# nyenyu12/BioInformatics-project-for-Shotgun-Metagenomics-Pseudo-alignment-shotgun-

Hardware: AMD Instinct MI355X
Metric: reads/sec pseudo-aligned (k=31, 150bp) at 1/2/4/8 GPUs; % HBM roofline (higher is better)
Workload: dtype u8

## Files before the change

### bioinformatics-project-for-shotgun-metagenomics-pseudo-alignment-shotgun-_amd/csrc/pa_align.hip

```cpp
#include <hip/hip_runtime.h>

#include <algorithm>
#include <cstdio>
#include <cstdlib>
#include <cstring>
#include <vector>

#include "pa_device.h"
#include "pa_internal.h"

using namespace pad;

namespace {

constexpr int kBlock = 256;
constexpr int kWaves = kBlock / 64;
constexpr uint32_t kSegMaxWaves = 16384;
constexpr uint64_t kSegSlack = 64ull * kSegMaxWaves;
constexpr uint32_t kLdsGenomeCap = 2048;

enum : uint32_t { F_MRQ = 1, F_MKQ = 2, F_MG = 4 };

struct AlignArgs {
    const void *table;
    uint64_t cap;
    HomeCfg home;
    uint32_t G;
    int k;
    const uint32_t *class_genomes;
    const uint64_t *class_mask;
    const uint32_t *tile_cls;
    const uint64_t *tile_pk;
    uint64_t tile_n;
    const uint64_t *goff;
    const uint64_t *tile_lw;
    const uint64_t *tile_big;
    const void *tile_nb;
    uint64_t nb_base1, nb_split;
    const uint32_t *nbbig_ld;
    uint64_t nbbig_mask;
    int nb_spec;
// ... 21 lines not shown
    unsigned long long *stats;
    unsigned long long *uniq;
    unsigned long long *amb;
    unsigned long long *first;
    uint32_t *queue;
    unsigned long long *qcount;
    unsigned long long *deferred_total;
    uint32_t *queue_hard;
    unsigned long long *queue_hard_count;
    uint32_t *queue_na;
    unsigned long long *queue_na_count;
    uint64_t *queue_na_keys;
    uint32_t *queue_rc;
    uint64_t *queue_rc_anc;
    unsigned long long *queue_rc_count;
    uint32_t *queue_na2;
    unsigned long long *queue_na2_count;
    uint64_t na_min;
    uint32_t na_seg;
    uint32_t *seg_cnt;
    uint32_t nseg;
    uint64_t seg_cap;
    uint64_t queue_cap;
    const uint4 *qmask;
    const uint8_t *qdrop;
    const uint32_t *rlist;
    const unsigned long long *rlist_count;
    unsigned long long *dbg;
};

__device__ __forceinline__ uint64_t first_key(uint64_t read, uint32_t rank) { return (read << 20) | rank; }


struct WgCounters {
    uint32_t *uniq;
    uint32_t *amb;
    unsigned long long *first;
    bool lds;
};

__device__ __forceinline__ void count_genome(const AlignArgs &a, const WgCounters &c, uint32_t g, bool unique,
                                             uint32_t times, uint64_t key) {
    if (c.lds) {
        atomicAdd(unique ? &c.uniq[g] : &c.amb[g], times);
        if (key < c.first[g]) atomicMin(&c.first[g], (unsigned long long)key);
    } else {
// ... 106 lines not shown
    }
    switch (k >> 2) {
        case 0: quality_reads<0>(qual, off, n, k, T, mrq, flags, qmask, qdrop); break;
        case 1: quality_reads<1>(qual, off, n, k, T, mrq, flags, qmask, qdrop); break;
        case 2: quality_reads<2>(qual, off, n, k, T, mrq, flags, qmask, qdrop); break;
        case 3: quality_reads<3>(qual, off, n, k, T, mrq, flags, qmask, qdrop); break;
        case 4: quality_reads<4>(qual, off, n, k, T, mrq, flags, qmask, qdrop); break;
        case 5: quality_reads<5>(qual, off, n, k, T, mrq, flags, qmask, qdrop); break;
        case 6: quality_reads<6>(qual, off, n, k, T, mrq, flags, qmask, qdrop); break;
        case 7: quality_reads<7>(qual, off, n, k, T, mrq, flags, qmask, qdrop); break;
        case 8: quality_reads<8>(qual, off, n, k, T, mrq, flags, qmask, qdrop); break;
        case 9: quality_reads<9>(qual, off, n, k, T, mrq, flags, qmask, qdrop); break;
        case 10: quality_reads<10>(qual, off, n, k, T, mrq, flags, qmask, qdrop); break;
        case 11: quality_reads<11>(qual, off, n, k, T, mrq, flags, qmask, qdrop); break;
        case 12: quality_reads<12>(qual, off, n, k, T, mrq, flags, qmask, qdrop); break;
        case 13: quality_reads<13>(qual, off, n, k, T, mrq, flags, qmask, qdrop); break;
        case 14: quality_reads<14>(qual, off, n, k, T, mrq, flags, qmask, qdrop); break;
        case 15: quality_reads<15>(qual, off, n, k, T, mrq, flags, qmask, qdrop); break;
        default: break;
    }
}

#include "pa_lane.h"

__global__ __launch_bounds__(256) void k_tile_big(const uint32_t *__restrict__ tile_cls, uint64_t n, uint32_t G,
                                                  const uint32_t *__restrict__ class_genomes, int32_t mg,
                                                  uint64_t *__restrict__ big, uint64_t n_words) {
    const uint32_t lane = threadIdx.x & 63;
    const uint64_t nw = (uint64_t)gridDim.x * (blockDim.x >> 6);
    for (uint64_t j = (uint64_t)blockIdx.x * (blockDim.x >> 6) + (threadIdx.x >> 6); j < n_words; j += nw) {
        const uint64_t t = 64 * j + lane;
        const uint32_t v = t < n ? tile_cls[t] : NONE;
        const bool ok = v != NONE && (int64_t)class_size_of(v & ~PA_TILE_REP, G, class_genomes) > (int64_t)mg;
        const uint64_t b = __ballot(ok);
        if (lane == 0) big[j] = b;
    }
}


__global__ __launch_bounds__(256) void k_nb_merge(const uint64_t *__restrict__ nb, const uint32_t *__restrict__ nbbig,
                                                  uint64_t n_words, uint4 *__restrict__ out) {
    const uint64_t stride = (uint64_t)gridDim.x * blockDim.x;
    for (uint64_t i = (uint64_t)blockIdx.x * blockDim.x + threadIdx.x; i < n_words; i += stride) {
        const uint64_t v = nb[i];
        out[i] = make_uint4((uint32_t)v, (uint32_t)(v >> 32), nbbig[i], 0u);
    }
// ... 427 lines not shown
    hipStream_t st;
    int slot;
    hipEvent_t e0 = nullptr;
    KernelTimer(pa_index *i, hipStream_t s, int sl) : idx(i), st(s), slot(sl) {
        if (idx && idx->profile && hipEventCreate(&e0) == hipSuccess) hipEventRecord(e0, st);
    }
    ~KernelTimer() {
        hipEvent_t e1 = nullptr;
        if (e0 && hipEventCreate(&e1) == hipSuccess && hipEventRecord(e1, st) == hipSuccess)
            idx->kev.push_back({slot, e0, e1});
        else if (e0)
            hipEventDestroy(e0);
    }
};

constexpr uint64_t kRcnbMinReads = 32768;
pa_status launch_lane(const AlignArgs &a0, hipStream_t st, pa_index *prof = nullptr, bool long_reads = false,
                      int nw = 1) {
    const bool need_q = (a0.prm.flags & (F_MRQ | F_MKQ)) != 0;
    const bool win_q = (a0.prm.flags & F_MKQ) != 0;
    const bool mg = (a0.prm.flags & F_MG) != 0;
    const bool nm4 = long_reads && !win_q && nw == 1;
    AlignArgs a = a0;
    const size_t shm = lane_lds_bytes(a.G, nm4 ? 4 : 2);
    auto kern = nw == 3
                    ? (win_q ? (mg ? k_align_lane<true, true, true, 2, 3> : k_align_lane<true, true, false, 2, 3>)
                       : need_q ? (mg ? k_align_lane<true, false, true, 2, 3> : k_align_lane<true, false, false, 2, 3>)
                                : (mg ? k_align_lane<false, false, true, 2, 3> : k_align_lane<false, false, false, 2, 3>))
              : nw == 2
                    ? (win_q ? (mg ? k_align_lane<true, true, true, 2, 2> : k_align_lane<true, true, false, 2, 2>)
                       : need_q ? (mg ? k_align_lane<true, false, true, 2, 2> : k_align_lane<true, false, false, 2, 2>)
                                : (mg ? k_align_lane<false, false, true, 2, 2> : k_align_lane<false, false, false, 2, 2>))
              : nm4 ? (need_q ? (mg ? k_align_lane<true, false, true, 4> : k_align_lane<true, false, false, 4>)
                              : (mg ? k_align_lane<false, false, true, 4> : k_align_lane<false, false, false, 4>))
              : win_q ? (mg ? k_align_lane<true, true, true> : k_align_lane<true, true, false>)
              : need_q ? (mg ? k_align_lane<true, false, true> : k_align_lane<true, false, false>)
                       : (mg ? k_align_lane<false, false, true> : k_align_lane<false, false, false>);
    if (shm > 64 * 1024) PA_HIP(hipFuncSetAttribute((const void *)kern, hipFuncAttributeMaxDynamicSharedMemorySize, (int)shm));
    int per_cu = 0, dev = 0, cus = 256;
    PA_HIP(hipOccupancyMaxActiveBlocksPerMultiprocessor(&per_cu, kern, kBlock, shm));
    PA_HIP(hipGetDevice(&dev));
    PA_HIP(hipDeviceGetAttribute(&cus, hipDeviceAttributeMultiprocessorCount, dev));
    const uint64_t want = (a.n + kBlock - 1) / kBlock;
    const uint64_t resident = (uint64_t)std::max(1, per_cu) * (uint64_t)cus;
    const unsigned grid = (unsigned)std::max<uint64_t>(1, std::min<uint64_t>(want, resident));
    {
        const char *e = std::getenv("PA_NA_SEG");
        const uint64_t waves = (uint64_t)grid * kWaves, chunks = (a.n + 63) / 64;
        a.nseg = (uint32_t)waves;
        a.seg_cap = 64 * ((chunks + waves - 1) / waves);
        a.na_seg = a.queue_na && a.queue_na_keys && a.seg_cnt && !nm4 && nw == 1 && waves <= kSegMaxWaves &&
                   waves * a.seg_cap <= a.queue_cap && !(e && e[0] == '0');
    }
    {
        KernelTimer kt(prof, st, PA_PROF_LANE);
        hipLaunchKernelGGL(kern, dim3(grid), dim3(kBlock), shm, st, a);
        PA_HIP(hipGetLastError());
    }
    if (a.queue_na) {
        AlignArgs b = a;
        if (prof && prof->rcnb_pending && a.queue_na_keys) {
            unsigned long long c = 0;
            PA_HIP(hipMemcpyAsync(&c, a.queue_na_count, 8, hipMemcpyDeviceToHost, st));
            PA_HIP(hipStreamSynchronize(st));
            if (c >= std::max<uint64_t>(kRcnbMinReads, a.n / 64)) {
                PA_TRY(pa::index_build_rcnb(prof, st));
                const char *e = std::getenv("PA_NA_RCNB");
                if (!(e && e[0] == '0')) b.tile_rcnb = prof->tile_rcnb;
            } else if (++prof->rcnb_checks >= 2) {
                prof->rcnb_pending = 0;
            }
        }
        if (a.queue_na_keys) {
// ... 179 lines not shown
}

pa_status reserve_queues(pa_index *idx, uint64_t n) {
    if (!idx->seg_cnt) PA_HIP(pa::dev_malloc(&idx->seg_cnt, (uint64_t)kSegMaxWaves * 4));
    n += kSegSlack;
    if (idx->queue_cap >= n) return PA_OK;
    pa::dev_free(idx->queue);
    pa::dev_free(idx->queue_hard);
    pa::dev_free(idx->queue_na);
    pa::dev_free(idx->queue_na2);
    pa::dev_free(idx->queue_na_keys);
    pa::dev_free(idx->queue_rc);
    pa::dev_free(idx->queue_rc_anc);
    idx->queue = idx->queue_hard = idx->queue_na = idx->queue_na2 = idx->queue_rc = nullptr;
    idx->queue_na_keys = idx->queue_rc_anc = nullptr;
    idx->queue_cap = 0;
    PA_HIP(pa::dev_malloc(&idx->queue, n * 4));
    PA_HIP(pa::dev_malloc(&idx->queue_hard, n * 4));
    PA_HIP(pa::dev_malloc(&idx->queue_na, n * 4));
    PA_HIP(pa::dev_malloc(&idx->queue_na2, n * 4));
    PA_HIP(pa::dev_malloc(&idx->queue_na_keys, n * 16));
    PA_HIP(pa::dev_malloc(&idx->queue_rc, n * 4));
    PA_HIP(pa::dev_malloc(&idx->queue_rc_anc, n * 8));
    if (!idx->na_count) PA_HIP(pa::dev_malloc(&idx->na_count, 24));
    idx->queue_cap = n;
    return PA_OK;
}

__global__ __launch_bounds__(256) void k_reads_qstats(const uint8_t *__restrict__ qual,
                                                      const uint64_t *__restrict__ off, uint64_t n, uint32_t *out) {
    typedef unsigned short us2 __attribute__((ext_vector_type(2)));
    const uint64_t tid = (uint64_t)blockIdx.x * blockDim.x + threadIdx.x, stride = (uint64_t)gridDim.x * blockDim.x;
    const uint64_t b0 = off[0], b1 = off[n];
    const uint64_t mis = (uint64_t)(uintptr_t)qual & 15;
    const uint64_t a0 = min(b1, ((b0 + mis + 15) & ~15ull) - mis), a1 = max(a0, ((b1 + mis) & ~15ull) - mis);
    uint32_t qm = 255, lm = 0xFFFFFFFFu;
    if (tid < 16) {
        if (b0 + tid < a0) qm = min(qm, (uint32_t)qual[b0 + tid]);
        if (a1 + tid < b1) qm = min(qm, (uint32_t)qual[a1 + tid]);
    }
    us2 mlo = {255, 255}, mhi = {255, 255};
    const uint4 *vp = (const uint4 *)(qual + a0);
    const uint64_t nv = (a1 - a0) >> 4;
    auto fold = [&](const uint4 x) {
        const uint32_t d[4] = {x.x, x.y, x.z, x.w};
#pragma unroll
        for (int j = 0; j < 4; j++) {
// ... 166 lines not shown
                hipLaunchKernelGGL(idx->k > 63 ? k_quality_masks<true> : k_quality_masks<false>, dim3((unsigned)std::min<uint64_t>((r->n + 255) / 256, 65536)),
                                   dim3(256), 0, st, r->qual, r->off, r->n, (int)idx->k, (int64_t)a.prm.mrq,
                                   (int64_t)a.prm.mkq, a.prm.flags & (F_MRQ | F_MKQ), idx->qmask, idx->qdrop);
                PA_HIP(hipGetLastError());
                a.qmask = idx->qmask;
                a.qdrop = idx->qdrop;
            }
            bool na = a.bloom != nullptr;
            if (const char *e = std::getenv("PA_LANE_NOANCHOR")) na = e[0] == '1';
            if (idx->nw > 3) na = false;
            a.queue_na = na ? idx->queue_na : nullptr;
            a.queue_na_count = idx->na_count;
            const bool rcw = na && a.tile_rcp && a.bloom;
            a.queue_na_keys = rcw ? idx->queue_na_keys : nullptr;
            a.queue_rc = idx->queue_rc;
            a.queue_rc_anc = idx->queue_rc_anc;
            a.queue_rc_count = idx->na_count + 1;
            a.seg_cnt = idx->seg_cnt;
            a.queue_cap = idx->queue_cap;
            a.queue_na2 = idx->queue_na2;
            a.queue_na2_count = idx->na_count + 2;
            a.na_min = 32768;
            if (const char *e = std::getenv("PA_NA_MIN")) a.na_min = std::strtoull(e, nullptr, 10);
            if (na) PA_HIP(hipMemsetAsync(idx->na_count, 0, 24, st));
            const bool long_reads = r->max_len > (uint32_t)kLaneMaxLen ||
                                    (r->max_len >= idx->k && r->max_len - idx->k + 1 > (uint32_t)kLaneMaxW);
            PA_TRY(launch_lane(a, st, idx, long_reads, idx->nw));
            a.rlist = idx->queue_hard;
            a.rlist_count = a.queue_hard_count;
        }
        {
            KernelTimer kt(idx, st, PA_PROF_WAVE);
            PA_TRY(idx->nw == 1   ? launch_fast_wpl<1>(a, wpl, st)
                   : idx->nw == 2 ? launch_fast_wpl<2>(a, wpl, st)
                   : idx->nw == 3 ? launch_fast_wpl<3>(a, wpl, st)
                                  : launch_fast_wpl<4>(a, wpl, st));
        }
        if (idx->profile) {
            PA_HIP(hipEventRecord(e1, st));
            idx->ev_start.push_back(e0);
            idx->ev_stop.push_back(e1);
        }
        x.a = a;
        x.use_queue = 1;
    } else {
        x.use_queue = 0;
    }
// ... 113 lines not shown
```

### bioinformatics-project-for-shotgun-metagenomics-pseudo-alignment-shotgun-_amd/csrc/pa_lane.h

```cpp

constexpr uint64_t kPosMask = (1ull << 40) - 1;
template <int NM>
struct LaneShape {
    static constexpr int MAXW = 64 * NM;
    static constexpr int NWD = NM == 2 ? 6 : 9;
    static constexpr int MAXLEN = 32 * NWD - 16;
    static constexpr int NB = NM + 1;
};
constexpr int kLaneMaxW = LaneShape<2>::MAXW;
constexpr int kLaneMaxLen = LaneShape<2>::MAXLEN;
constexpr int kLaneWords = LaneShape<2>::NWD;
#ifndef PA_LANE_MAXMIS
#define PA_LANE_MAXMIS 40
#endif
constexpr uint32_t kLaneMaxMis = PA_LANE_MAXMIS;
#ifndef PA_LANE_PROBES
#define PA_LANE_PROBES 4
#endif
#ifndef PA_LANE_SEEDS
#define PA_LANE_SEEDS 5
#endif
#ifndef PA_SEED_SLOTS
#define PA_SEED_SLOTS 2
#endif
#ifndef PA_LANE_RANK_WORDS
#define PA_LANE_RANK_WORDS 6
#endif
#ifndef PA_LANE_SLOTS
#define PA_LANE_SLOTS 1
#endif
constexpr int kPassEntries = 64 * PA_LANE_PROBES;
#ifndef PA_TWO_WINQ
#define PA_TWO_WINQ 1
#endif
#ifndef PA_LANE_LDS_GENOMES
#define PA_LANE_LDS_GENOMES 1664
#endif
constexpr uint32_t kLaneLdsGenomeCap = PA_LANE_LDS_GENOMES;

template <int NM>
struct __align__(16) LaneWave {
    uint64_t R[64][LaneShape<NM>::NWD + 1];
    unsigned long long cand[64];
    uint32_t flags[64];
    uint32_t hr[64];
    uint32_t gsp[64];
    uint16_t list[kPassEntries];
    uint32_t again_r[128];
    unsigned long long again_a[128];
};

enum : int {
    LANE_UNIQUE = 0, LANE_AMB = 1, LANE_UNMAPPED = 2, LANE_DROP = 3, LANE_HARD = 4, LANE_WALK = 5, LANE_AGAIN = 6,
    LANE_NOANCHOR = 7
};

template <int N>
__device__ __forceinline__ uint64_t word_at(const uint64_t (&v)[N], uint32_t q) {
    uint64_t r = 0;
#pragma unroll
    for (int i = 0; i < N; i++) r = (q == (uint32_t)i) ? v[i] : r;
// ... 203 lines not shown
    }
}

template <int NWD = kLaneWords>
__device__ __forceinline__ uint32_t lane_count_mismatches(const uint64_t *row, uint32_t len, uint64_t A,
                                                          const uint64_t (&gw)[NWD + 1]) {
    const uint32_t gr = (uint32_t)(2 * A & 63);
    uint32_t n = 0;
    const uint32_t qlast = (len - 1) >> 5, rl = len - 32 * qlast;
    const uint64_t tail = rl >= 32 ? ~0ull : ~0ull << (64 - 2 * rl);
#pragma unroll
    for (int i = 0; i < NWD; i++) {
        if (32 * i >= (int)len) break;
        const uint64_t gwi = gr ? ((gw[i] << gr) | (gw[i + 1] >> (64 - gr))) : gw[i];
        uint64_t d = row[i] ^ gwi;
        if ((uint32_t)i == qlast) d &= tail;
        n += __popcll((d | (d >> 1)) & 0x5555555555555555ull);
    }
    return n;
}

__device__ __forceinline__ bool lane_fits(const AlignArgs &a, uint32_t len, int64_t A) {
    return A >= 0 && (uint64_t)A + len <= a.tile_n;
}

template <int NM, bool NEED_Q, bool WIN_Q, bool SEEDS = true, int NW = 1>
__device__ __forceinline__ void lane_prep(const AlignArgs &a, uint64_t r, unsigned long long cd, uint64_t *row,
                                          LaneRead<NM> &S) {
    using SH = LaneShape<NM>;
    static_assert(NM == 2 || !WIN_Q, "the window-quality masks cover 128 windows");
    constexpr int NWD = SH::NWD;
    S.kind = LANE_HARD;
    S.hr = S.nspec = S.nincl = 0;
#pragma unroll
    for (int i = 0; i < NM; i++) S.F[i] = 0;
    S.qf = 0;
    S.uoff = 0;
    const int k = a.k;
    const uint32_t flags = a.prm.flags;
    const uint64_t o = a.off[r];
    const uint32_t len = (uint32_t)(a.off[r + 1] - o);
    const uint64_t o0 = o & ~15ull;
    const uint32_t shift = (uint32_t)(o & 15);
    S.len = len;
    if (len > (uint32_t)SH::MAXLEN) return (void)LANE_HARD_WHY(0);
    if (NEED_Q) {
// ... 256 lines not shown
    uint64_t gw[kLaneWords + 1], pa3[3], pb3[3];
    lane_blocks<true>(a, Ac, len, gw, pa3, pb3);
    const uint32_t g = S.acls < a.G ? S.acls : genome_of(a.goff, a.gblk, atp);
    S.g = g;
    const uint64_t gs = a.goff[g], ge = a.goff[g + 1];
    if (!in_tile || A < (int64_t)gs || (uint64_t)A + W - 1 + k > ge) {
        S.kind = LANE_HARD;
        return (void)LANE_HARD_WHY(4);
    }
    const uint32_t fr = (uint32_t)(Ac & 63);
    const uint64_t PA0 = fr ? (pa3[0] >> fr) | (pa3[1] << (64 - fr)) : pa3[0];
    const uint64_t PA1 = fr ? (pa3[1] >> fr) | (pa3[2] << (64 - fr)) : pa3[1];
    const uint64_t PB0 = fr ? (pb3[0] >> fr) | (pb3[1] << (64 - fr)) : pb3[0];
    const uint64_t PB1 = fr ? (pb3[1] >> fr) | (pb3[2] << (64 - fr)) : pb3[1];
    const uint64_t IX0 = PA0 | PB0, IX1 = PA1 | PB1;
    uint64_t U0 = 0, U1 = 0, V0 = 0, V1 = 0, NP0 = 0, NP1 = 0, NS0 = 0, NS1 = 0, NG0 = 0, NG1 = 0;
    uint32_t nmis = 0;
    const bool has_nb = a.tile_nb != nullptr;
    uint64_t epk = 0;
    uint32_t cpk = 0;
    uint32_t nnb = 0;
    const uint32_t qlast = (len - 1) >> 5, rl = len - 32 * qlast;
    const uint64_t tail = rl >= 32 ? ~0ull : ~0ull << (64 - 2 * rl);
#pragma unroll
    for (int i = 0; i < kLaneWords; i++) {
        if (32 * i >= (int)len) break;
        const uint64_t gwi = gr ? ((gw[i] << gr) | (gw[i + 1] >> (64 - gr))) : gw[i];
        uint64_t d = row[i] ^ gwi;
        if ((uint32_t)i == qlast) d &= tail;
        uint64_t m = (d | (d >> 1)) & 0x5555555555555555ull;
        while (m) {
            const uint32_t j = __builtin_clzll(m) >> 1, e = 32 * i + j;
            m &= ~(1ull << (62 - 2 * j));
            const int32_t lo = (int32_t)e - k + 1 < 0 ? 0 : (int32_t)e - k + 1;
            const int32_t hi = (int32_t)e < (int32_t)W - 1 ? (int32_t)e : (int32_t)W - 1;
            if (lo > hi) continue;
            const uint64_t r0 = lo < 64 ? ((~0ull << lo) & (hi >= 63 ? ~0ull : ((2ull << hi) - 1))) : 0ull;
            const uint64_t r1 =
                hi >= 64 ? ((lo <= 64 ? ~0ull : (~0ull << (lo - 64))) & (hi >= 127 ? ~0ull : ((2ull << (hi - 64)) - 1)))
                         : 0ull;
            if (!((r0 & IX0) | (r1 & IX1))) continue;
            if (++nmis > 8) {
                if (nmis > kLaneMaxMis) {
                    S.kind = LANE_HARD;
                    return (void)LANE_HARD_WHY(5);
                }
                V0 |= r0;
                V1 |= r1;
                U0 |= r0;
                U1 |= r1;
                continue;
            }
            V0 |= U0 & r0;
            V1 |= U1 & r1;
            U0 |= r0;
            U1 |= r1;
            if (has_nb) {
                const uint32_t cg = (uint32_t)(gwi >> (62 - 2 * j)) & 3u, cr = (uint32_t)(row[i] >> (62 - 2 * j)) & 3u;
                epk |= (uint64_t)e << (8 * nnb);
                cpk |= ((cr - cg - 1) & 3u) << (2 * nnb);
                nnb++;
            }
        }
    }
#pragma unroll 1
    for (uint32_t b0 = 0; b0 < nnb; b0 += 4) {
        uint64_t nv[4];
        uint32_t ng[4];
        int32_t sf[4];
#pragma unroll
        for (int u = 0; u < 4; u++) {
            const uint32_t q = b0 + u < nnb ? b0 + u : b0;
            const uint32_t e = (uint32_t)(epk >> (8 * q)) & 255u, c = (cpk >> (2 * q)) & 3u;
            const uint64_t ni = 3 * ((uint64_t)A + e) + c;
            uint64_t v8;
            if constexpr (NW == 3) {
                const uint64_t p = (uint64_t)A + e;
                v8 = (((const uint32_t *)a.tile_nb)[p >> 3] >> (4 * (p & 7) + c)) & 1u;
                nv[u] = v8;
            } else if constexpr (NW == 2) {
                v8 = ((const uint64_t *)a.tile_nb)[ni];
                nv[u] = v8;
            } else if (MG && a.tile_nbm) {
                const uint4 v = a.tile_nbm[ni];
                nv[u] = (uint64_t)v.x | ((uint64_t)v.y << 32);
                ng[u] = v.z;
            } else {
// ... 475 lines not shown

#ifndef PA_LANE_WAVES_Q
#define PA_LANE_WAVES_Q 4
#endif
#ifndef PA_LANE_WAVES_LONG
#define PA_LANE_WAVES_LONG 4
#endif
#ifndef PA_LANE_WAVES_MG
#define PA_LANE_WAVES_MG 4
#endif
#ifndef PA_LANE_WAVES_W
#define PA_LANE_WAVES_W 3
#endif
template <bool NEED_Q, bool WIN_Q, bool MG, int NM = 2, int NW = 1>
__global__ __launch_bounds__(kBlock) __attribute__((amdgpu_waves_per_eu(
    NM == 4 ? PA_LANE_WAVES_LONG
            : (NW >= 2 ? PA_LANE_WAVES_W : (WIN_Q ? PA_LANE_WAVES_Q : (MG ? PA_LANE_WAVES_MG : PA_LANE_WAVES))))))
void k_align_lane(AlignArgs a) {
    using LW_t = LaneWave<NM>;
    constexpr int NWD = LaneShape<NM>::NWD;
    extern __shared__ __align__(16) unsigned char smem[];
    const uint32_t G = a.G;
    const int lane = lane_id();
    const bool lds = G <= kLaneLdsGenomeCap;
    const size_t cnt_bytes = lds ? ((size_t)G * 8 + 15) / 16 * 16 : 0;
    uint32_t *first = (uint32_t *)smem;
    uint32_t *uniq = first + (lds ? G : 0);
    LW_t &LW = ((LW_t *)(smem + cnt_bytes))[__builtin_amdgcn_readfirstlane(threadIdx.x >> 6)];
    if (lds) {
        for (uint32_t i = threadIdx.x; i < G; i += kBlock) {
            first[i] = ~0u;
            uniq[i] = 0;
        }
        __syncthreads();
    }
    uint32_t n_uniq = 0, n_amb = 0, n_unm = 0, n_drop = 0;
    uint64_t n_hr = 0, n_qf = 0;
    LW.R[lane][NWD] = 0;
    const uint64_t n_chunks = (a.n + 63) / 64, wave_stride = (uint64_t)gridDim.x * kWaves;
    uint64_t chunk = (uint64_t)blockIdx.x * kWaves + (uint32_t)__builtin_amdgcn_readfirstlane(threadIdx.x >> 6);
    const uint32_t wave_id = (uint32_t)chunk;
    const uint64_t seg_base = (uint64_t)wave_id * a.seg_cap;
    uint32_t seg_na = 0;
    uint32_t n_again = 0;
    while (true) {
        uint32_t r = ~0u;
        unsigned long long cd = ~0ull;
        bool again_batch = false;
        if (n_again >= 64 || (chunk >= n_chunks && n_again > 0)) {
            const uint32_t take = n_again < 64 ? n_again : 64;
            if ((uint32_t)lane < take) {
                r = LW.again_r[n_again - take + lane];
                cd = LW.again_a[n_again - take + lane];
            }
            n_again -= take;
            again_batch = true;
        } else if (chunk < n_chunks) {
            r = chunk * 64 + lane < a.n ? (uint32_t)(chunk * 64 + lane) : ~0u;
            chunk += wave_stride;
        } else {
            break;
        }
        LaneRead<NM> S;
        S.kind = LANE_UNMAPPED + 100;
        wave_sync();
        auto my_row = [&]() -> uint64_t * {
            uint32_t l = (uint32_t)lane;
            asm volatile("" : "+v"(l));
            return LW.R[l];
        };
        if (r != ~0u) lane_prep<NM, NEED_Q, WIN_Q, true, NW>(a, r, cd, my_row(), S);
#if defined(PA_STATS) || defined(PA_DISSECT)
        if (a.dbg_mode == 10 && S.kind == LANE_WALK) S.kind = LANE_AMB;
#endif
#pragma unroll 1
        for (int attempt = again_batch ? 1 : 0; attempt < 2; attempt++) {
            if (S.kind == LANE_WALK) {
                if constexpr (NM == 2)
                    lane_walk_150<WIN_Q, MG, NW>(a, my_row(), S);
                else
                    if constexpr (NM == 4 && !WIN_Q && NW == 1 && PA_LANE_HALVES)
                        lane_walk_halves<MG>(a, my_row(), S);
                    else
                        lane_walk_long<NM, WIN_Q, MG>(a, my_row(), S);
            }
#if defined(PA_STATS) || defined(PA_DISSECT)
            if (a.dbg_mode == 11 && S.kind == LANE_WALK) S.kind = LANE_AMB;
#endif
            if (!__ballot(S.kind == LANE_WALK)) break;
            if (S.kind == LANE_WALK && S.nspec > 0 && (!MG || (a.mg_nb && !lane_any(S.P)))) {
                const int64_t X = (int64_t)(lane_popc(S.P) + S.uoff);
                const int64_t ns = (int64_t)S.nspec;
                if (ns >= X + (a.prm.m > 0 ? a.prm.m : 1) && (a.prm.p < 0 || X - ns <= a.prm.p)) {
                    S.kind = LANE_UNIQUE;
// ... 119 lines not shown
        if (WIN_Q) n_qf += wave_sum(settled ? S.qf : 0u);
    }
    if (lane == 0) {
        if (NM == 2 && a.na_seg) {
            a.seg_cnt[wave_id] = seg_na;
            if (seg_na) atomicAdd(a.queue_na_count, (unsigned long long)seg_na);
        }
        if (n_uniq) atomicAdd(&a.stats[0], (unsigned long long)n_uniq);
        if (n_amb) atomicAdd(&a.stats[1], (unsigned long long)n_amb);
        if (n_unm) atomicAdd(&a.stats[2], (unsigned long long)n_unm);
        if (n_drop) atomicAdd(&a.stats[3], (unsigned long long)n_drop);
        if (n_hr && MG) atomicAdd(&a.stats[5], (unsigned long long)n_hr);
        if (WIN_Q && n_qf) atomicAdd(&a.stats[4], (unsigned long long)n_qf);
    }
    if (lds) {
        __syncthreads();
        for (uint32_t i = threadIdx.x; i < G; i += kBlock) {
            if (uniq[i]) atomicAdd(&a.uniq[i], (unsigned long long)uniq[i]);
            if (first[i] != ~0u) atomicMin(&a.first[i], (unsigned long long)first_key(a.base + first[i], 0));
        }
    }
}

constexpr size_t lane_lds_bytes(uint32_t G, int NM = 2) {
    return (G <= kLaneLdsGenomeCap ? ((size_t)G * 8 + 15) / 16 * 16 : 0) +
           (size_t)kWaves * (NM == 4 ? sizeof(LaneWave<4>) : sizeof(LaneWave<2>));
}

#ifndef PA_NA_GROUP
#define PA_NA_GROUP 8
#endif
__device__ __forceinline__ uint64_t bits128(uint64_t x0, uint64_t x1, int s) {
    return s == 0 ? x0 : ((x0 << s) | (x1 >> (64 - s)));
}
template <int NAG, int KC, bool CARRY = true>
__device__ __forceinline__ uint32_t bloom_group(const AlignArgs &a, const uint64_t *row, uint32_t w0, uint32_t act,
                                                bool fresh, uint32_t &prev_blk, uint4 &cur, bool &cur_mm,
                                                uint4 (*hc)[kBlock]) {
    static_assert(NAG == 8 || NAG == 16, "a group's bases are 128 bits from a multiple of 16");
    const int k = KC ? KC : a.k, sh = 64 - 2 * k;
    const int mm = k < 15 ? k : 15;
    const int S = k - mm + 1;
    const uint32_t o = 2 * w0, q = o >> 6, r = o & 63;
    uint64_t X0 = row[q], X1 = row[q + 1];
    if (r) {
        const uint64_t X2 = row[q + 2];
        X0 = (X0 << r) | (X1 >> (64 - r));
        X1 = (X1 << r) | (X2 >> (64 - r));
// ... 656 lines not shown
```

Before: 3.902 billion.

## Add dynamic chunk claiming and prefetched read offsets to the lane kernel

Replaces the static grid-stride chunk assignment in the lane align kernel with atomic work claiming, where each wave takes runs of chunks from a global counter for load balance. It also prefetches the next chunk's read offsets into per-wave LDS while the current chunk packs, and splits lane_prep into lane_pack and lane_seeds so the prefetch and claim can be issued late. The mismatch scan is rewritten as a single loop over packed masks. In exchange it gives up some LDS genome capacity, needs larger queue slack per segment, and adds an atomic per claim.

```diff
diff --git a/bioinformatics-project-for-shotgun-metagenomics-pseudo-alignment-shotgun-_amd/csrc/pa_align.hip b/bioinformatics-project-for-shotgun-metagenomics-pseudo-alignment-shotgun-_amd/csrc/pa_align.hip
--- a/bioinformatics-project-for-shotgun-metagenomics-pseudo-alignment-shotgun-_amd/csrc/pa_align.hip
+++ b/bioinformatics-project-for-shotgun-metagenomics-pseudo-alignment-shotgun-_amd/csrc/pa_align.hip
@@ -16,7 +16,8 @@
 constexpr int kBlock = 256;
 constexpr int kWaves = kBlock / 64;
 constexpr uint32_t kSegMaxWaves = 16384;
-constexpr uint64_t kSegSlack = 64ull * kSegMaxWaves;
+constexpr uint32_t kSegSlackWaves = 8192, kSegSlackChunks = 5;
+constexpr uint64_t kSegSlack = 64ull * kSegSlackChunks * kSegSlackWaves;
 constexpr uint32_t kLdsGenomeCap = 2048;
 
 enum : uint32_t { F_MRQ = 1, F_MKQ = 2, F_MG = 4 };
@@ -84,6 +85,7 @@
     uint32_t nseg;
     uint64_t seg_cap;
     uint64_t queue_cap;
+    uint32_t *lane_next;
     const uint4 *qmask;
     const uint8_t *qdrop;
     const uint32_t *rlist;
@@ -236,6 +238,7 @@
 }
 
 #include "pa_lane.h"
+static_assert(kSegSlackChunks >= 1 + kLaneClaimHeld, "the queues' slack covers the chunks a wave holds");
 
 __global__ __launch_bounds__(256) void k_tile_big(const uint32_t *__restrict__ tile_cls, uint64_t n, uint32_t G,
                                                   const uint32_t *__restrict__ class_genomes, int32_t mg,
@@ -709,7 +712,7 @@
     const bool mg = (a0.prm.flags & F_MG) != 0;
     const bool nm4 = long_reads && !win_q && nw == 1;
     AlignArgs a = a0;
-    const size_t shm = lane_lds_bytes(a.G, nm4 ? 4 : 2);
+    const size_t shm = lane_lds_bytes(a.G, nm4 ? 4 : 2, lane_sched(win_q, mg, nm4 ? 4 : 2, nw));
     auto kern = nw == 3
                     ? (win_q ? (mg ? k_align_lane<true, true, true, 2, 3> : k_align_lane<true, true, false, 2, 3>)
                        : need_q ? (mg ? k_align_lane<true, false, true, 2, 3> : k_align_lane<true, false, false, 2, 3>)
@@ -730,12 +733,14 @@
     PA_HIP(hipDeviceGetAttribute(&cus, hipDeviceAttributeMultiprocessorCount, dev));
     const uint64_t want = (a.n + kBlock - 1) / kBlock;
     const uint64_t resident = (uint64_t)std::max(1, per_cu) * (uint64_t)cus;
-    const unsigned grid = (unsigned)std::max<uint64_t>(1, std::min<uint64_t>(want, resident));
+    unsigned grid = (unsigned)std::max<uint64_t>(1, std::min<uint64_t>(want, resident));
+    if (const char *e = std::getenv("PA_LANE_GRID"))
+        grid = (unsigned)std::max<uint64_t>(1, std::min<uint64_t>(grid, std::strtoull(e, nullptr, 10)));
     {
         const char *e = std::getenv("PA_NA_SEG");
         const uint64_t waves = (uint64_t)grid * kWaves, chunks = (a.n + 63) / 64;
         a.nseg = (uint32_t)waves;
-        a.seg_cap = 64 * ((chunks + waves - 1) / waves);
+        a.seg_cap = 64 * ((chunks + waves - 1) / waves + kLaneClaimHeld);
         a.na_seg = a.queue_na && a.queue_na_keys && a.seg_cnt && !nm4 && nw == 1 && waves <= kSegMaxWaves &&
                    waves * a.seg_cap <= a.queue_cap && !(e && e[0] == '0');
     }
@@ -961,7 +966,7 @@
     PA_HIP(pa::dev_malloc(&idx->queue_na_keys, n * 16));
     PA_HIP(pa::dev_malloc(&idx->queue_rc, n * 4));
     PA_HIP(pa::dev_malloc(&idx->queue_rc_anc, n * 8));
-    if (!idx->na_count) PA_HIP(pa::dev_malloc(&idx->na_count, 24));
+    if (!idx->na_count) PA_HIP(pa::dev_malloc(&idx->na_count, 32));
     idx->queue_cap = n;
     return PA_OK;
 }
@@ -1174,7 +1179,8 @@
             a.queue_na2_count = idx->na_count + 2;
             a.na_min = 32768;
             if (const char *e = std::getenv("PA_NA_MIN")) a.na_min = std::strtoull(e, nullptr, 10);
-            if (na) PA_HIP(hipMemsetAsync(idx->na_count, 0, 24, st));
+            a.lane_next = (uint32_t *)(idx->na_count + 3);
+            if (na || PA_LANE_CLAIM) PA_HIP(hipMemsetAsync(idx->na_count, 0, 32, st));
             const bool long_reads = r->max_len > (uint32_t)kLaneMaxLen ||
                                     (r->max_len >= idx->k && r->max_len - idx->k + 1 > (uint32_t)kLaneMaxW);
             PA_TRY(launch_lane(a, st, idx, long_reads, idx->nw));
diff --git a/bioinformatics-project-for-shotgun-metagenomics-pseudo-alignment-shotgun-_amd/csrc/pa_lane.h b/bioinformatics-project-for-shotgun-metagenomics-pseudo-alignment-shotgun-_amd/csrc/pa_lane.h
--- a/bioinformatics-project-for-shotgun-metagenomics-pseudo-alignment-shotgun-_amd/csrc/pa_lane.h
+++ b/bioinformatics-project-for-shotgun-metagenomics-pseudo-alignment-shotgun-_amd/csrc/pa_lane.h
@@ -33,10 +33,33 @@
 #ifndef PA_TWO_WINQ
 #define PA_TWO_WINQ 1
 #endif
+#ifndef PA_LANE_CLAIM
+#define PA_LANE_CLAIM 1
+#endif
+#ifndef PA_LANE_PREOFF
+#define PA_LANE_PREOFF 1
+#endif
+#ifndef PA_LANE_RUN
+#define PA_LANE_RUN 2
+#endif
+constexpr uint32_t kLaneClaimHeld = PA_LANE_CLAIM ? 2 + PA_LANE_RUN : 0;
+#ifndef PA_LANE_TOPWAIT
+#define PA_LANE_TOPWAIT 1
+#endif
+#ifndef PA_LANE_LATE
+#define PA_LANE_LATE 1
+#endif
+constexpr int kLaneWaitVm0 = 0x0F70;
+constexpr bool lane_sched(bool win_q, bool mg, int nm, int nw) {
+    return (PA_LANE_CLAIM || PA_LANE_PREOFF) && nm == 2 && (nw > 1 || !mg);
+}
+constexpr size_t kLaneOffsBytes = 66 * 8;
 #ifndef PA_LANE_LDS_GENOMES
 #define PA_LANE_LDS_GENOMES 1664
 #endif
-constexpr uint32_t kLaneLdsGenomeCap = PA_LANE_LDS_GENOMES;
+constexpr uint32_t lane_lds_genome_cap(bool sched) {
+    return sched && PA_LANE_PREOFF ? PA_LANE_LDS_GENOMES - 264 : PA_LANE_LDS_GENOMES;
+}
 
 template <int NM>
 struct __align__(16) LaneWave {
@@ -286,6 +309,236 @@
 
 __device__ __forceinline__ bool lane_fits(const AlignArgs &a, uint32_t len, int64_t A) {
     return A >= 0 && (uint64_t)A + len <= a.tile_n;
+}
+
+template <int NM, bool NEED_Q, bool WIN_Q, class AHEAD>
+__device__ __forceinline__ bool lane_pack(const AlignArgs &a, uint64_t r, uint64_t o, uint64_t o1, uint64_t *row,
+                                          LaneRead<NM> &S, AHEAD &&ahead) {
+    using SH = LaneShape<NM>;
+    static_assert(NM == 2 || !WIN_Q, "the window-quality masks cover 128 windows");
+    constexpr int NWD = SH::NWD;
+    S.kind = LANE_HARD;
+    S.hr = S.nspec = S.nincl = 0;
+#pragma unroll
+    for (int i = 0; i < NM; i++) S.F[i] = 0;
+    S.qf = 0;
+    S.uoff = 0;
+    const int k = a.k;
+    const uint32_t len = (uint32_t)(o1 - o);
+    const uint64_t o0 = o & ~15ull;
+    const uint32_t shift = (uint32_t)(o & 15);
+    S.len = len;
+    if (len > (uint32_t)SH::MAXLEN) return LANE_HARD_WHY(0), false;
+    if (NEED_Q) {
+        if (a.qdrop[r]) {
+            S.kind = LANE_DROP;
+            return false;
+        }
+        if (WIN_Q) {
+            const uint4 m = a.qmask[r];
+            S.F[0] = (uint64_t)m.x | ((uint64_t)m.y << 32);
+            S.F[NM - 1] = (uint64_t)m.z | ((uint64_t)m.w << 32);
+            S.qf = (uint32_t)(__popcll(S.F[0]) + __popcll(S.F[NM - 1]));
+        }
+    }
+    if (len < (uint32_t)k) {
+        S.kind = LANE_UNMAPPED;
+        return false;
+    }
+    const uint32_t W = len - k + 1;
+    S.W = W;
+    if (W > (uint32_t)SH::MAXW) return LANE_HARD_WHY(0), false;
+    const uint4 *sp = (const uint4 *)(a.seq + o0);
+    const uint32_t s2 = 2 * shift;
+    uint32_t bad = 0;
+    uint64_t prev = 0;
+    constexpr int CG = NM == 2 ? 2 * NWD : 6;
+#pragma unroll
+    for (int g0 = 0; g0 < 2 * NWD; g0 += CG) {
+    uint4 ch[CG];
+#pragma unroll
+    for (int c = 0; c < CG; c++)
+        ch[c] = (g0 + c < 2 * NWD && 16u * (g0 + c) < shift + len)
+                    ? sp[g0 + c]
+                    : make_uint4(0x41414141u, 0x41414141u, 0x41414141u, 0x41414141u);
+    if (g0 == 0) ahead();
+#pragma unroll
+    for (int q = g0 / 2; q < (g0 + CG) / 2 && q < NWD; q++) {
+        uint64_t P = 0;
+        if (32u * q < shift + len) {
+            const uint4 v0 = ch[2 * q - g0], v1 = ch[2 * q + 1 - g0];
+            const uint32_t d[8] = {v0.x, v0.y, v0.z, v0.w, v1.x, v1.y, v1.z, v1.w};
+#pragma unroll
+            for (int e = 0; e < 8; e++) {
+                const uint32_t cd = swar_codes(d[e]);
+#ifdef PA_PACK_MASKED
+                bad |= swar_bad_bytes(d[e], cd) & in_read_mask(32 * q + 4 * e, shift, len);
+#else
+                bad |= swar_bad_bytes(d[e], cd);
+#endif
+                P |= (uint64_t)swar_pack_byte(cd) << (56 - 8 * e);
+            }
+        }
+        if (q > 0) row[q - 1] = s2 ? ((prev << s2) | (P >> (64 - s2))) : prev;
+        prev = P;
+    }
+    }
+    row[NWD - 1] = prev << s2;
+#ifndef PA_PACK_MASKED
+    if (bad) {
+        bad = 0;
+#pragma unroll 1
+        for (int c = 0; c < 2 * NWD; c++) {
+            if (16u * c >= shift + len) break;
+            const uint4 v = sp[c];
+            const uint32_t d[4] = {v.x, v.y, v.z, v.w};
+#pragma unroll
+            for (int e = 0; e < 4; e++)
+                bad |= swar_bad_bytes(d[e], swar_codes(d[e])) & in_read_mask(16u * c + 4 * e, shift, len);
+        }
+    }
+#endif
+    if (bad) return LANE_HARD_WHY(2), false;
+#if defined(PA_STATS) || defined(PA_DISSECT)
+    if (a.dbg_mode == 13) {
+        S.kind = LANE_AMB;
+        return false;
+    }
+#endif
+    return true;
+}
+
+template <int NM, int NW = 1>
+__device__ __forceinline__ void lane_seeds(const AlignArgs &a, unsigned long long cd, const uint64_t *row,
+                                           LaneRead<NM> &S) {
+    const int k = a.k;
+    const uint32_t len = S.len, W = S.W;
+    if (cd != ~0ull) {
+        S.anc = cd;
+        S.acls = NONE;
+        S.kind = LANE_WALK;
+        return;
+    }
+    const int sh = 64 - 2 * k;
+    constexpr int NSEED = PA_LANE_SEEDS;
+    auto sw = [W](int i) { return (uint32_t)(((uint64_t)(W - 1) * (uint32_t)i) / (NSEED - 1)); };
+    uint64_t skey[NW == 1 ? NSEED : 1];
+    Key<NW> skk[NW == 1 ? 1 : NSEED];
+    if constexpr (NW == 1) {
+#pragma unroll
+        for (int i = 0; i < NSEED; i++) skey[i] = row_bits(row, 2 * sw(i)) >> sh;
+    } else {
+        (void)sh;
+#pragma unroll
+        for (int i = 0; i < NSEED; i++) skk[i] = row_key<NW>(row, sw(i), k);
+    }
+#ifndef PA_LANE_SEED_ROUNDS
+#define PA_LANE_SEED_ROUNDS 2
+#endif
+    uint32_t sfound = 0, scls[NSEED], stp32[NSEED];
+    {
+#ifndef PA_LANE_SEED_R1
+#define PA_LANE_SEED_R1 (1u | (1u << (NSEED - 1)))
+#endif
+        constexpr uint32_t all = (1u << NSEED) - 1, outer = PA_LANE_SEED_R1;
+        uint32_t act = PA_LANE_SEED_ROUNDS > 1 ? outer : all;
+#pragma unroll 1
+        for (int round = 0; round < 2 && act; round++) {
+            uint32_t f;
+            if constexpr (NW == 1)
+                lane_probe<NSEED, PA_SEED_SLOTS>(a, skey, act, f, scls, stp32);
+            else
+                lane_probe_k<NSEED, NW == 3 ? 1 : PA_SEED_SLOTS, NW>(a, skk, act, f, scls, stp32);
+            sfound |= f;
+            bool spec = false;
+#pragma unroll
+            for (int i = 0; i < NSEED; i++) spec |= bit(f, i) && cls_of(scls[i]) < a.G && stp32[i] != NONE;
+#ifndef PA_LANE_R2_ONLY_UNSEEDED
+#define PA_LANE_R2_ONLY_UNSEEDED 0
+#endif
+            act = (round == 0 && act != all && !spec && (!PA_LANE_R2_ONLY_UNSEEDED || f == 0)) ? all & ~outer : 0u;
+#if defined(PA_STATS) || defined(PA_DISSECT)
+            if (a.dbg_mode == 14) act = 0;
+#endif
+#ifdef PA_STATS
+            if (act) atomicAdd(&a.dbg[27], 1ull);
+#endif
+        }
+    }
+    uint64_t stp[NSEED];
+#pragma unroll
+    for (int i = 0; i < NSEED; i++) {
+        stp[i] = bit(sfound, i) && stp32[i] != NONE ? first_pos(scls[i], stp32[i], a.G, a.class_genomes, a.goff, a.tpos_local)
+                                                     : ~0ull;
+        scls[i] = cls_of(scls[i]);
+    }
+    int at = -1;
+#pragma unroll
+    for (int pass = 0; pass < 2; pass++)
+#pragma unroll
+        for (int i = 0; i < NSEED; i++)
+            if (at < 0 && stp[i] != ~0ull && (pass == 1 || scls[i] < a.G)) at = i;
+    if (at < 0) {
+        if (a.queue_na) S.kind = LANE_NOANCHOR;
+        if constexpr (NW == 1) {
+            S.P[0] = rc_key(skey[NSEED - 1], k);
+            S.P[1] = rc_key(skey[0], k);
+        }
+        return (void)LANE_HARD_WHY(3);
+    }
+    S.anc = stp[0] | ((uint64_t)sw(0) << 40);
+    S.acls = scls[0];
+#pragma unroll
+    for (int i = 1; i < NSEED; i++)
+        if (at == i) {
+            S.anc = stp[i] | ((uint64_t)sw(i) << 40);
+            S.acls = scls[i];
+        }
+    if (S.acls >= a.G) {
+        const int64_t e0 = (int64_t)(S.anc & kPosMask) - (int64_t)(S.anc >> 40);
+        int64_t e1 = INT64_MIN, e2 = INT64_MIN;
+        uint64_t t1 = 0, t2 = 0;
+        uint32_t w1 = 0, c1 = 0, w2 = 0, c2 = 0;
+#pragma unroll
+        for (int i = 0; i < NSEED; i++) {
+            const int64_t Ai = (int64_t)stp[i] - sw(i);
+            if (stp[i] == ~0ull || Ai == e0 || Ai == e1 || e2 != INT64_MIN) continue;
+            if (e1 == INT64_MIN) {
+                e1 = Ai;
+                t1 = stp[i], w1 = sw(i), c1 = scls[i];
+            } else {
+                e2 = Ai;
+                t2 = stp[i], w2 = sw(i), c2 = scls[i];
+            }
+        }
+        if (e1 != INT64_MIN) {
+#ifdef PA_STATS
+            atomicAdd(&a.dbg[26], 1ull);
+#endif
+#ifndef PA_LANE_RANK_WORDS4
+#define PA_LANE_RANK_WORDS4 5
+#endif
+            constexpr int NR = NM == 2 ? PA_LANE_RANK_WORDS : PA_LANE_RANK_WORDS4;
+            const uint32_t rlen = len < 32u * NR ? len : 32u * NR;
+            const bool f0 = lane_fits(a, len, e0), f1 = lane_fits(a, len, e1), f2 = e2 != INT64_MIN && lane_fits(a, len, e2);
+            uint64_t g0[NR + 1], g1[NR + 1], g2[NR + 1], u3[3];
+            lane_blocks<false, NR>(a, f0 ? (uint64_t)e0 : 0, rlen, g0, u3, u3);
+            lane_blocks<false, NR>(a, f1 ? (uint64_t)e1 : 0, rlen, g1, u3, u3);
+            lane_blocks<false, NR>(a, f2 ? (uint64_t)e2 : 0, rlen, g2, u3, u3);
+            const uint32_t m0 = f0 ? lane_count_mismatches<NR>(row, rlen, (uint64_t)e0, g0) : ~0u;
+            const uint32_t m1 = f1 ? lane_count_mismatches<NR>(row, rlen, (uint64_t)e1, g1) : ~0u;
+            const uint32_t m2 = f2 ? lane_count_mismatches<NR>(row, rlen, (uint64_t)e2, g2) : ~0u;
+            uint32_t bj = 0, best = m0;
+            if (m1 < best) best = m1, bj = 1;
+            if (m2 < best) best = m2, bj = 2;
+            if (bj == 1) {
+                S.anc = t1 | ((uint64_t)w1 << 40), S.acls = c1;
+            } else if (bj == 2) {
+                S.anc = t2 | ((uint64_t)w2 << 40), S.acls = c2;
+            }
+        }
+    }
+    S.kind = LANE_WALK;
 }
 
 template <int NM, bool NEED_Q, bool WIN_Q, bool SEEDS = true, int NW = 1>
@@ -588,6 +841,76 @@
     uint32_t nnb = 0;
     const uint32_t qlast = (len - 1) >> 5, rl = len - 32 * qlast;
     const uint64_t tail = rl >= 32 ? ~0ull : ~0ull << (64 - 2 * rl);
+    auto mismatch = [&](uint32_t e, auto &&sub) -> bool {
+        const int32_t lo = (int32_t)e - k + 1 < 0 ? 0 : (int32_t)e - k + 1;
+        const int32_t hi = (int32_t)e < (int32_t)W - 1 ? (int32_t)e : (int32_t)W - 1;
+        if (lo > hi) return true;
+        const uint64_t r0 = lo < 64 ? ((~0ull << lo) & (hi >= 63 ? ~0ull : ((2ull << hi) - 1))) : 0ull;
+        const uint64_t r1 =
+            hi >= 64 ? ((lo <= 64 ? ~0ull : (~0ull << (lo - 64))) & (hi >= 127 ? ~0ull : ((2ull << (hi - 64)) - 1)))
+                     : 0ull;
+        if (!((r0 & IX0) | (r1 & IX1))) return true;
+        if (++nmis > 8) {
+            if (nmis > kLaneMaxMis) return false;
+            V0 |= r0;
+            V1 |= r1;
+            U0 |= r0;
+            U1 |= r1;
+            return true;
+        }
+        V0 |= U0 & r0;
+        V1 |= U1 & r1;
+        U0 |= r0;
+        U1 |= r1;
+        if (has_nb) {
+            epk |= (uint64_t)e << (8 * nnb);
+            cpk |= sub() << (2 * nnb);
+            nnb++;
+        }
+        return true;
+    };
+#ifndef PA_LANE_ONELOOP
+#define PA_LANE_ONELOOP 1
+#endif
+#if PA_LANE_ONELOOP
+    constexpr int NP2 = (kLaneWords + 1) / 2;
+    uint64_t MM[NP2];
+#pragma unroll
+    for (int p = 0; p < NP2; p++) MM[p] = 0;
+#pragma unroll
+    for (int i = 0; i < kLaneWords; i++) {
+        if (32 * i >= (int)len) break;
+        const uint64_t gwi = gr ? ((gw[i] << gr) | (gw[i + 1] >> (64 - gr))) : gw[i];
+        uint64_t d = row[i] ^ gwi;
+        if ((uint32_t)i == qlast) d &= tail;
+        const uint64_t m = (d | (d >> 1)) & 0x5555555555555555ull;
+        MM[i >> 1] |= (i & 1) ? m << 1 : m;
+    }
+    while (true) {
+        uint64_t mm = 0;
+        uint32_t p = 0;
+#pragma unroll
+        for (int q = NP2 - 1; q >= 0; q--)
+            if (MM[q]) mm = MM[q], p = (uint32_t)q;
+        if (!mm) break;
+        const uint64_t ev = mm & 0x5555555555555555ull;
+        const uint32_t odd = ev ? 0u : 1u;
+        const uint32_t j = __builtin_clzll(odd ? mm >> 1 : ev) >> 1, e = 32 * (2 * p + odd) + j;
+        const uint64_t clr = ~((odd ? 2ull : 1ull) << (62 - 2 * j));
+#pragma unroll
+        for (int q = 0; q < NP2; q++) MM[q] &= p == (uint32_t)q ? clr : ~0ull;
+        const bool ok = mismatch(e, [&]() {
+            const uint32_t o = gr + 2 * e;
+            const uint32_t cg = (uint32_t)(word_at(gw, o >> 6) >> (62 - (o & 63))) & 3u;
+            const uint32_t cr = (uint32_t)(row[e >> 5] >> (62 - 2 * (e & 31))) & 3u;
+            return (cr - cg - 1) & 3u;
+        });
+        if (!ok) {
+            S.kind = LANE_HARD;
+            return (void)LANE_HARD_WHY(5);
+        }
+    }
+#else
 #pragma unroll
     for (int i = 0; i < kLaneWords; i++) {
         if (32 * i >= (int)len) break;
@@ -598,37 +921,17 @@
         while (m) {
             const uint32_t j = __builtin_clzll(m) >> 1, e = 32 * i + j;
             m &= ~(1ull << (62 - 2 * j));
-            const int32_t lo = (int32_t)e - k + 1 < 0 ? 0 : (int32_t)e - k + 1;
-            const int32_t hi = (int32_t)e < (int32_t)W - 1 ? (int32_t)e : (int32_t)W - 1;
-            if (lo > hi) continue;
-            const uint64_t r0 = lo < 64 ? ((~0ull << lo) & (hi >= 63 ? ~0ull : ((2ull << hi) - 1))) : 0ull;
-            const uint64_t r1 =
-                hi >= 64 ? ((lo <= 64 ? ~0ull : (~0ull << (lo - 64))) & (hi >= 127 ? ~0ull : ((2ull << (hi - 64)) - 1)))
-                         : 0ull;
-            if (!((r0 & IX0) | (r1 & IX1))) continue;
-            if (++nmis > 8) {
-                if (nmis > kLaneMaxMis) {
-                    S.kind = LANE_HARD;
-                    return (void)LANE_HARD_WHY(5);
-                }
-                V0 |= r0;
-                V1 |= r1;
-                U0 |= r0;
-                U1 |= r1;
-                continue;
-            }
-            V0 |= U0 & r0;
-            V1 |= U1 & r1;
-            U0 |= r0;
-            U1 |= r1;
-            if (has_nb) {
+            const bool ok = mismatch(e, [&]() {
                 const uint32_t cg = (uint32_t)(gwi >> (62 - 2 * j)) & 3u, cr = (uint32_t)(row[i] >> (62 - 2 * j)) & 3u;
-                epk |= (uint64_t)e << (8 * nnb);
-                cpk |= ((cr - cg - 1) & 3u) << (2 * nnb);
-                nnb++;
-            }
-        }
-    }
+                return (cr - cg - 1) & 3u;
+            });
+            if (!ok) {
+                S.kind = LANE_HARD;
+                return (void)LANE_HARD_WHY(5);
+            }
+        }
+    }
+#endif
 #pragma unroll 1
     for (uint32_t b0 = 0; b0 < nnb; b0 += 4) {
         uint64_t nv[4];
@@ -1150,11 +1453,16 @@
     extern __shared__ __align__(16) unsigned char smem[];
     const uint32_t G = a.G;
     const int lane = lane_id();
-    const bool lds = G <= kLaneLdsGenomeCap;
+    constexpr bool kSched = lane_sched(WIN_Q, MG, NM, NW);
+    const bool lds = G <= lane_lds_genome_cap(kSched);
     const size_t cnt_bytes = lds ? ((size_t)G * 8 + 15) / 16 * 16 : 0;
     uint32_t *first = (uint32_t *)smem;
     uint32_t *uniq = first + (lds ? G : 0);
     LW_t &LW = ((LW_t *)(smem + cnt_bytes))[__builtin_amdgcn_readfirstlane(threadIdx.x >> 6)];
+    uint64_t *noff = nullptr;
+    if constexpr (kSched && PA_LANE_PREOFF)
+        noff = (uint64_t *)(smem + cnt_bytes + kWaves * sizeof(LW_t) +
+                            kLaneOffsBytes * (uint32_t)__builtin_amdgcn_readfirstlane(threadIdx.x >> 6));
     if (lds) {
         for (uint32_t i = threadIdx.x; i < G; i += kBlock) {
             first[i] = ~0u;
@@ -1165,12 +1473,29 @@
     uint32_t n_uniq = 0, n_amb = 0, n_unm = 0, n_drop = 0;
     uint64_t n_hr = 0, n_qf = 0;
     LW.R[lane][NWD] = 0;
+    constexpr bool CLAIM = PA_LANE_CLAIM && kSched, PREOFF = PA_LANE_PREOFF && kSched;
     const uint64_t n_chunks = (a.n + 63) / 64, wave_stride = (uint64_t)gridDim.x * kWaves;
     uint64_t chunk = (uint64_t)blockIdx.x * kWaves + (uint32_t)__builtin_amdgcn_readfirstlane(threadIdx.x >> 6);
+    uint64_t chunk1 = chunk + wave_stride;
+    auto chunk_offs = [&](uint64_t c, uint64_t &o0, uint64_t &o1) {
+        const uint64_t i = c * 64 + (uint32_t)lane;
+        o1 = a.off[i + 1 < a.n ? i + 1 : a.n];
+        if (lane == 0) o0 = a.off[i];
+    };
+    if constexpr (PREOFF) {
+        if (chunk < n_chunks) {
+            uint64_t o0 = 0, o1;
+            chunk_offs(chunk, o0, o1);
+            noff[lane + 1] = o1;
+            if (lane == 0) noff[0] = o0;
+        }
+    }
     const uint32_t wave_id = (uint32_t)chunk;
     const uint64_t seg_base = (uint64_t)wave_id * a.seg_cap;
     uint32_t seg_na = 0;
     uint32_t n_again = 0;
+    uint64_t res = 0;
+    uint32_t nres = 0;
     while (true) {
         uint32_t r = ~0u;
         unsigned long long cd = ~0ull;
@@ -1185,10 +1510,35 @@
             again_batch = true;
         } else if (chunk < n_chunks) {
             r = chunk * 64 + lane < a.n ? (uint32_t)(chunk * 64 + lane) : ~0u;
-            chunk += wave_stride;
+            if constexpr (!CLAIM && !PREOFF) chunk += wave_stride;
         } else {
             break;
         }
+        const bool fresh = !again_batch;
+        uint32_t cl = 0;
+        uint64_t no0 = 0, no1 = 0;
+        bool claimed = false;
+        if constexpr ((CLAIM || PREOFF) && PA_LANE_TOPWAIT) __builtin_amdgcn_s_waitcnt(kLaneWaitVm0);
+        uint32_t run = 1;
+        if constexpr (CLAIM) {
+            claimed = fresh && nres == 0 && chunk1 < n_chunks &&
+                      (!(NM == 2 && a.na_seg) || seg_na + 64 * kLaneClaimHeld <= a.seg_cap);
+            if (PA_LANE_RUN > 1 && chunk1 + 4 * wave_stride < n_chunks) run = PA_LANE_RUN;
+        }
+        bool ahead_done = !fresh;
+        auto ahead = [&]() {
+            if (ahead_done) return;
+            ahead_done = true;
+            if (PREOFF && chunk1 < n_chunks) chunk_offs(chunk1, no0, no1);
+            if constexpr (CLAIM) {
+                if (claimed && lane == 0) {
+                    uint32_t z = 0;
+                    asm volatile("" : "+v"(z));
+                    cl = atomicAdd(a.lane_next + z, run);
+                }
+            }
+        };
+        if constexpr (!PA_LANE_LATE) ahead();
         LaneRead<NM> S;
         S.kind = LANE_UNMAPPED + 100;
         wave_sync();
@@ -1197,7 +1547,48 @@
             asm volatile("" : "+v"(l));
             return LW.R[l];
         };
-        if (r != ~0u) lane_prep<NM, NEED_Q, WIN_Q, true, NW>(a, r, cd, my_row(), S);
+        if constexpr (!CLAIM && !PREOFF) {
+            if (r != ~0u) lane_prep<NM, NEED_Q, WIN_Q, true, NW>(a, r, cd, my_row(), S);
+        } else {
+            bool packed = false;
+            if (r != ~0u) {
+                uint64_t o = 0, o1 = 0;
+                if constexpr (PREOFF) {
+                    o = noff[lane], o1 = noff[lane + 1];
+                    asm volatile("" : "+v"(o), "+v"(o1));
+                }
+                if (!PREOFF || !fresh) {
+                    o = a.off[r], o1 = a.off[r + 1];
+                    if constexpr (PREOFF) asm volatile("" : "+v"(o), "+v"(o1));
+                }
+                packed = lane_pack<NM, NEED_Q, WIN_Q>(a, r, o, o1, my_row(), S, ahead);
+            }
+            ahead();
+            if (fresh) {
+                if constexpr (PREOFF) {
+                    wave_sync();
+                    if (chunk1 < n_chunks) {
+                        noff[lane + 1] = no1;
+                        if (lane == 0) noff[0] = no0;
+                    }
+                }
+                chunk = chunk1;
+                if constexpr (CLAIM) {
+                    if (nres) {
+                        chunk1 = res++;
+                        nres--;
+                    } else if (claimed) {
+                        chunk1 = 2 * wave_stride + (uint32_t)__builtin_amdgcn_readfirstlane(cl);
+                        res = chunk1 + 1;
+                        nres = run - 1;
+                    } else {
+                        chunk1 = ~0ull;
+                    }
+                } else
+                    chunk1 += wave_stride;
+            }
+            if (packed) lane_seeds<NM, NW>(a, cd, my_row(), S);
+        }
 #if defined(PA_STATS) || defined(PA_DISSECT)
         if (a.dbg_mode == 10 && S.kind == LANE_WALK) S.kind = LANE_AMB;
 #endif
@@ -1363,8 +1754,9 @@
     }
 }
 
-constexpr size_t lane_lds_bytes(uint32_t G, int NM = 2) {
-    return (G <= kLaneLdsGenomeCap ? ((size_t)G * 8 + 15) / 16 * 16 : 0) +
+constexpr size_t lane_lds_bytes(uint32_t G, int NM = 2, bool sched = false) {
+    return (G <= lane_lds_genome_cap(sched) ? ((size_t)G * 8 + 15) / 16 * 16 : 0) +
+           (sched && PA_LANE_PREOFF ? kWaves * kLaneOffsBytes : 0) +
            (size_t)kWaves * (NM == 4 ? sizeof(LaneWave<4>) : sizeof(LaneWave<2>));
 }
 
```

Result: faster. 4.313 billion, median of 6 (+10.5%).
